# olof3/QuantumOptimalControl.jl

Hardware: AMD Instinct MI355X
Metric: GRAPE gradient evals/sec (dim N, T slices, B seeds) @ 1/2/4/8 GPU (higher is better)
Workload: dtype f64

## Files before the change

quantumoptimalcontrol.jl_amd/csrc/qoc_blkseg.hpp:

```cpp
#pragma once
#include "qoc_blku.hpp"

namespace qoc {

struct BlksegParams {
  double rad[3];
  double mur[3], mui[3];
  double theta_cap;
  int S;
  int L;
  int UPW;
  int RB;
  const double* u;
  double* u_copy;
  double* u_copy2;
  double* J2;
  cx<double>* coef2;
  double* dJdu;
  unsigned long long* terms;
  unsigned int* done;
  double* best;
  long long seed_offset;
  double* best_res;
  double* best_out;
  double2* gseg;
  const int* stale;
  const double2* gtab;
  double pen_mu;
  unsigned int prow[3];
  unsigned int pcol;
  double2* dseg;
};
enum { BLKSEG_FUSED = 0, BLKSEG_FWD = 1, BLKSEG_BWD = 2 };

__host__ __device__ inline size_t blkseg_off_rec(int NB, int nblk) { return (size_t)6 * NB * NB * nblk; }
__host__ __device__ inline size_t blkseg_off_slot(int NB, int nblk, int Nt) { return blkseg_off_rec(NB, nblk) + 4 * (size_t)Nt; }
__host__ __device__ inline size_t blkseg_off_g0(int NB, int nblk, int Nt, int S) {
  return blkseg_off_slot(NB, nblk, Nt) + (size_t)2 * S * NB * NB * nblk;
}
__host__ __device__ inline size_t blkseg_off_xN(int NB, int nblk, int Nt, int S) {
  return blkseg_off_g0(NB, nblk, Nt, S) + (size_t)2 * NB * NB * nblk;
}
__host__ __device__ inline size_t blkseg_off_xt(int N, int m, int NB, int nblk, int Nt, int S) {
  return blkseg_off_xN(NB, nblk, Nt, S) + (size_t)2 * N * m;
}
__host__ __device__ inline size_t blkseg_off_cf(int N, int m, int NB, int nblk, int Nt, int S) {
  return blkseg_off_xt(N, m, NB, nblk, Nt, S) + (size_t)2 * N * m;
}
// ... 17 lines not shown
constexpr size_t BLKSEG_LDS_MAX = (size_t)160 * 1024;
__host__ __device__ inline int blkseg_rb(int upw, int nu) {
  const int r = 64 / (upw * (nu > 0 ? nu : 1));
  return r < 1 ? 1 : r > 4 ? 4 : r;
}

#ifdef QOC_PROBE
static __device__ unsigned long long g_segw[32];
#define SEGW_SET(slot, v)                                                        \
  do {                                                                           \
    if (blockIdx.x == 7 && (threadIdx.x & 63) == 0) g_segw[slot] = (v);          \
  } while (0)
static __device__ int g_seg_noturn, g_seg_turnmode;
#define SEG_TURNS (!g_seg_noturn)
#define SEG_TURNMODE g_seg_turnmode
#else
#define SEG_TURNS true
#define SEG_TURNMODE 1
#define SEGW_SET(slot, v) \
  do {                    \
  } while (0)
#endif


template <int NB, bool AH, bool BH>
__device__ __forceinline__ void seg_mm(const double (&ar)[NB * NB], const double (&ai)[NB * NB], const double (&br)[NB * NB],
                                       const double (&bi)[NB * NB], double (&cr)[NB * NB], double (&ci)[NB * NB]) {
#pragma unroll
  for (int i = 0; i < NB; ++i)
#pragma unroll
    for (int k = 0; k < NB; ++k) {
      double sr = 0.0, si = 0.0;
#pragma unroll
      for (int q = 0; q < NB; ++q) {
        const int ea = AH ? q * NB + i : i * NB + q, eb = BH ? k * NB + q : q * NB + k;
// ... 218 lines not shown
  st = T.s[K];
#pragma unroll
  for (int k = K - 1; k >= 0; --k) {
    ct = fma(ct, t2, T.c[k]);
    st = fma(st, t2, T.s[k]);
  }
  st *= t;
}
template <int K = BLKSEG_KMAX>
__device__ __forceinline__ void sk2_z(const Sk2& g0, const double* rec, double& zr, double& zi) {
  double ct, st;
  sk2_phase<K>(g0.d0, g0.d1, ct, st);
  const double2 ph = *reinterpret_cast<const double2*>(rec);
  zr = ph.x * ct - ph.y * st;
  zi = fma(ph.x, st, ph.y * ct);
}
template <int K = BLKSEG_KMAX, bool EX = false>
__device__ __forceinline__ void sk2_form(const Sk2 (&g)[3], double2 ph, double2 u, Sk2& ah, double (&ur)[4],
                                         double (&ui)[4], double* ex = nullptr) {
  constexpr BlksegTrig T = blkseg_trig();
  ah.d0 = fma(u.y, g[2].d0, fma(u.x, g[1].d0, g[0].d0));
  ah.d1 = fma(u.y, g[2].d1, fma(u.x, g[1].d1, g[0].d1));
  ah.r = fma(u.y, g[2].r, fma(u.x, g[1].r, g[0].r));
  ah.q = fma(u.y, g[2].q, fma(u.x, g[1].q, g[0].q));
  const double a = 0.5 * (ah.d0 - ah.d1);
  const double w = fma(a, a, fma(ah.r, ah.r, ah.q * ah.q));
  double cw = T.c[K], sw = T.s[K], s3 = EX ? T.d[K] : 0.0, ct, st;
#pragma unroll
  for (int k = K - 1; k >= 0; --k) {
    cw = fma(cw, w, T.c[k]);
// ... 262 lines not shown
    Lr[e] = Rr[e] = er * vr - ei * vi;
    Li[e] = Ri[e] = fma(er, vi, ei * vr);
  }
  acc1 = acc2 = 0.0;
  seg_trace<NB>(genf(), Lr, Li, 1.0, m1r, m1i, m2r, m2i, acc1, acc2);
  double f = 1.0;
#pragma unroll 1
  for (int n = 1; n < nex; ++n) {
    seg_rx<NB>(Rr, Ri, xr_, xi_);
    seg_xlr<NB>(Lr, Li, Rr, Ri, xr_, xi_);
    f /= (double)(n + 1);
    seg_trace<NB>(genf(), Lr, Li, f, m1r, m1i, m2r, m2i, acc1, acc2);
  }
}

__device__ __forceinline__ double block_max(double v, double* scratch) {
  for (int off = 32; off > 0; off >>= 1) v = fmax(v, __shfl_xor(v, off));
  const int w = threadIdx.x >> 6, l = threadIdx.x & 63;
  __syncthreads();
  if (l == 0) scratch[w] = v;
  __syncthreads();
  double s = scratch[0];
  const int nw = (blockDim.x + 63) >> 6;
  for (int i = 1; i < nw; ++i) s = fmax(s, scratch[i]);
  __syncthreads();
  return s;
}

__device__ __forceinline__ void wave_lds_sync() {
  __builtin_amdgcn_fence(__ATOMIC_RELEASE, "wavefront");
  __builtin_amdgcn_wave_barrier();
  __builtin_amdgcn_fence(__ATOMIC_ACQUIRE, "wavefront");
}

__device__ __forceinline__ void seg_turn(int grp, int ngrp, int jj) {
  if ((grp + jj) % ngrp == 0) __builtin_amdgcn_s_setprio(1);
  else __builtin_amdgcn_s_setprio(0);
}
template <bool DEFER>
struct SegProg {
  int* prog;
  int partner, other;
  bool on, young;
// ... 57 lines not shown
  }
#pragma unroll
  for (int i = 0; i < NB; ++i)
#pragma unroll
    for (int j = 0; j < NB; ++j) {
      double sr = 0.0, si = 0.0;
#pragma unroll
      for (int q = 0; q < NB; ++q) {
        sr = fma(ur[q * NB + i], tr[q * NB + j], fma(ui[q * NB + i], ti[q * NB + j], sr));
        si = fma(ur[q * NB + i], ti[q * NB + j], fma(-ui[q * NB + i], tr[q * NB + j], si));
      }
      dp[(i * NB + j) * stride] = make_double2(sr, si);
    }
}

template <int NB, int ORD, int WMAX, int MODE = BLKSEG_FUSED, bool PEN = false>
__global__ __launch_bounds__(64 * WMAX) void k_blkseg_eval(const TChainArgs g, const BlkArgs bk, const BlksegParams sp) {
  extern __shared__ __attribute__((aligned(16))) unsigned char smem[];
  if constexpr (MODE == BLKSEG_BWD) {
    if (sp.stale && *sp.stale != 0) return;
  }
  constexpr int E = NB * NB;
  constexpr bool GREG = NB == 2 && WMAX <= 8;
  constexpr bool XA = NB == 2;
  constexpr int NV1 = NB == 2 ? 2 : 1;
  const int N = g.N, m = g.m, nu = g.nu, Nt = g.Nt, nblk = bk.nblk, S = sp.S, L = sp.L;
  const int tid = threadIdx.x, nthr = blockDim.x, w = tid >> 6, l = tid & 63, W = nthr >> 6;
  const int b = blockIdx.x;
  const size_t Nm = (size_t)N * m;
  BK_T(t0);
  double* const lds = reinterpret_cast<double*>(smem);
  double2* const gsh = reinterpret_cast<double2*>(lds);
  double* const rec = lds + blkseg_off_rec(NB, nblk);
  double2* const slot = reinterpret_cast<double2*>(lds + blkseg_off_slot(NB, nblk, Nt));
  double2* const g0s = reinterpret_cast<double2*>(lds + blkseg_off_g0(NB, nblk, Nt, S));
  double* const xN = lds + blkseg_off_xN(NB, nblk, Nt, S);
  double2* const xtl = reinterpret_cast<double2*>(lds + blkseg_off_xt(N, m, NB, nblk, Nt, S));
  cx<double>* const cf = reinterpret_cast<cx<double>*>(lds + blkseg_off_cf(N, m, NB, nblk, Nt, S));
  double* const red = lds + blkseg_off_red(N, m, NB, nblk, Nt, S);
  double* const wred = lds + blkseg_off_wred(N, m, NB, nblk, Nt, S);
  const int RB = sp.RB;
  double* const dJ = lds + blkseg_off_dJ(N, m, NB, nblk, Nt, S, W, RB);
  double2* const d0s = reinterpret_cast<double2*>(lds + blkseg_off_d0(N, m, nu, NB, nblk, Nt, S, W, RB));

  const int uw = l / nblk;
// ... 6 lines not shown
      for (int i = 0; i < NB; ++i) pm |= (int)((sp.prow[i] >> beta) & 1u) << i;
  }
  constexpr int PE = PEN ? NB * NB : 1;
  const int ntab = 3 * E * nblk;
  const double2* const x0g = reinterpret_cast<const double2*>(g.x0) + (g.x0_per_seed ? (size_t)b * Nm : 0);
  const double2* const xtg = reinterpret_cast<const double2*>(g.Xt);
  const double* ub = sp.u + (size_t)b * Nt * nu;
  const bool u16 = nu == 2 && (reinterpret_cast<size_t>(ub) & 15) == 0;
  auto load_u = [&](int k) -> double2 {
    if (u16) return reinterpret_cast<const double2*>(ub)[k];
    return make_double2(nu > 0 ? ub[(size_t)k * nu] : 0.0, nu > 1 ? ub[(size_t)k * nu + 1] : 0.0);
  };
  const bool hasx = MODE != BLKSEG_BWD && (size_t)tid < Nm;
  double2 tab0 = make_double2(0.0, 0.0), x00 = tab0, xt0 = tab0, ua = tab0, ubb = tab0;
  if (tid < ntab) tab0 = sp.gtab[tid];
  if (hasx) {
    x00 = x0g[tid];
    xt0 = xtg[tid];
  }
  if (tid < Nt) ua = load_u(tid);
  if (tid + nthr < Nt) ubb = load_u(tid + nthr);
  int brw[NB];
#pragma unroll
  for (int i = 0; i < NB; ++i) brw[i] = bk.brow[beta * NB + i];
  {
    if (tid < ntab) gsh[tid] = tab0;
    for (int q = tid + nthr; q < ntab; q += nthr) gsh[q] = sp.gtab[q];
    if constexpr (MODE != BLKSEG_BWD) {
      double2* const xN2 = reinterpret_cast<double2*>(xN);
      if (hasx) {
        xN2[tid] = x00;
        xtl[tid] = xt0;
      }
      for (size_t o = (size_t)tid + nthr; o < Nm; o += nthr) {
        xN2[o] = x0g[o];
        xtl[o] = xtg[o];
      }
    }
  }
  double rmax = 0.0;
  const bool cmu = sp.mur[1] == 0.0 && sp.mur[2] == 0.0 && sp.mui[1] == 0.0 && sp.mui[2] == 0.0;
  double2 emu0 = make_double2(1.0, 0.0);
  if (cmu) {
    const double er = exp(sp.mur[0]);
    double sn, cs;
    sincos(sp.mui[0], &sn, &cs);
    emu0 = make_double2(er * cs, er * sn);
  }
  auto slice = [&](int k, double2 uk) {
    const double u1 = uk.x, u2 = uk.y;
    for (int j = 0; j < nu; ++j) {
      const double v = j ? u2 : u1;
      if (sp.u_copy) sp.u_copy[((size_t)b * Nt + k) * nu + j] = v;
      if (sp.u_copy2) sp.u_copy2[((size_t)b * Nt + k) * nu + j] = v;
    }
    rmax = fmax(rmax, fma(fabs(u2), sp.rad[2], fma(fabs(u1), sp.rad[1], sp.rad[0])));
    double2* r = reinterpret_cast<double2*>(rec + 4 * (size_t)k);
    if (cmu) {
      r[0] = emu0;
    } else {
      const double mr = fma(u2, sp.mur[2], fma(u1, sp.mur[1], sp.mur[0]));
      const double mi = fma(u2, sp.mui[2], fma(u1, sp.mui[1], sp.mui[0]));
      const double er = exp(mr);
      double sn, cs;
      sincos(mi, &sn, &cs);
      r[0] = make_double2(er * cs, er * sn);
    }
    r[1] = make_double2(u1, u2);
  };
  if (tid < Nt) slice(tid, ua);
  if (tid + nthr < Nt) slice(tid + nthr, ubb);
  for (int k = tid + 2 * nthr; k < Nt; k += nthr) slice(k, load_u(k));
  rmax = block_max(rmax, red);
  int J = 0;
  double s0 = 1.0;
  while (rmax * s0 > sp.theta_cap && J < 60) {
    s0 *= 0.5;
    ++J;
  }
  int P = 0;
  {
    const double bb = rmax * s0, tol = 1.1102230246251565e-16;
    constexpr BlkuCoef K = blku_coef();
    double term = bb;
#pragma unroll
    for (int q = 0; q < BLKU_TMAX; ++q) {
      if (!(term > tol * fma(-bb, K.inv[q + 2], 1.0))) break;
      P = q + 1;
      term *= bb * K.inv[q + 2];
    }
  }
  P = __builtin_amdgcn_readfirstlane(P);
  J = __builtin_amdgcn_readfirstlane(J);
  int nex = 1;
  if constexpr (ORD == 0) nex = __builtin_amdgcn_readfirstlane(blkseg_exact_terms(rmax));
  if (tid < 8) reinterpret_cast<int*>(red + 24)[tid] = 0;
  if (J) {
    for (int k = tid; k < Nt; k += nthr) {
      rec[4 * (size_t)k + 2] *= s0;
      rec[4 * (size_t)k + 3] *= s0;
    }
  }
  __syncthreads();
  BK_T(t1);
  BK_ADD(0, t1 - t0);

  const int s = w * sp.UPW + uw;
  const bool sact = lact && s < S;
  const int kb = sact ? s * L : 0;
  const int ke = sact ? min(kb + L, Nt) : 0;
  double2 greg[GREG ? 3 : 1][GREG ? E : 1];
  if constexpr (GREG) {
#pragma unroll
    for (int j = 0; j < 3; ++j)
#pragma unroll
      for (int e = 0; e < E; ++e) greg[j][e] = gsh[(beta * 3 + j) * E + e];
  }
  auto gen_at = [&](int bc) {
// ... 24 lines not shown
  double Hr[PE], Hi[PE];
#pragma unroll
  for (int e = 0; e < PE; ++e) Hr[e] = Hi[e] = 0.0;
  const int Lf = Nt - (S - 1) * L;
  const bool fast = NB == 2 && J == 0;
  Sk2 gk[3];
  if constexpr (NB == 2) {
#pragma unroll
    for (int j = 0; j < 3; ++j) {
      double2 e4[4];
#pragma unroll
      for (int e = 0; e < 4; ++e) e4[e] = gsh[(beta * 3 + j) * E + e];
      gk[j] = sk2_of(e4);
    }
  }
  const bool zdl = NB != 2 || (gk[1].d0 == 0.0 && gk[1].d1 == 0.0 && gk[2].d0 == 0.0 && gk[2].d1 == 0.0);
  const bool zd = __syncthreads_and(zdl ? 1 : 0) != 0 && cmu && sp.mur[0] == 0.0;
  const double za0 = NB == 2 ? 0.5 * (gk[0].d0 - gk[0].d1) : 0.0;
  const int ksel = __builtin_amdgcn_readfirstlane(blkseg_series_k(rmax * s0));
  const bool su = fast && zd;
  double pq[4] = {1.0, 0.0, 0.0, 0.0};
  auto lane_z = [&](double& zr, double& zi) {
    zr = 1.0;
    zi = 0.0;
    if constexpr (NB == 2) {
      if (su) {
        if (ksel == 5) sk2_z<5>(gk[0], rec, zr, zi);
        else if (ksel == 7) sk2_z<7>(gk[0], rec, zr, zi);
        else sk2_z<BLKSEG_KMAX>(gk[0], rec, zr, zi);
      }
    }
  };
  const double* const reck = rec + 4 * (size_t)kb;
  auto p1_fast = [&](int jj, auto SEL_, auto K_, auto ZD_) {
    constexpr bool SEL = decltype(SEL_)::value;
    constexpr int KS = decltype(K_)::value;
    constexpr bool ZD = decltype(ZD_)::value;
    if constexpr (NB == 2) {
    if constexpr (ZD) {
      double vv[2][4];
      bool act[2];
#pragma unroll
      for (int v = 0; v < 2; ++v) {
        const int k = kb + jj + v;
// ... 57 lines not shown
      p1_fast(jj, std::true_type(), K_, ZD_);
    }
    if constexpr (NB == 2) {
      if constexpr (decltype(ZD_)::value) sk2_expand(pq, qr, qi);
    }
  };
  auto loop1 = [&](auto K_) {
    if (zd) loop1z(K_, std::true_type());
    else loop1z(K_, std::false_type());
  };
  double Gr[E], Gi[E];
  auto gseg_at = [&](int e) -> double2& { return sp.gseg[(((size_t)b * E + e) * S + s) * nblk + beta]; };
  auto dl_at = [&](int e) -> double2& { return slot[((size_t)s * E + e) * nblk + beta]; };
  auto dseg_at = [&](int e) -> double2& { return sp.dseg[(((size_t)b * E + e) * S + s) * nblk + beta]; };
  if constexpr (MODE == BLKSEG_BWD) {
#pragma unroll
    for (int e = 0; e < E; ++e) {
      const double2 v = sact ? gseg_at(e) : make_double2(0.0, 0.0);
      Gr[e] = v.x;
      Gi[e] = v.y;
    }
    if constexpr (PEN) {
      if (pm)
#pragma unroll
        for (int e = 0; e < E; ++e) dl_at(e) = dseg_at(e);
    }
    if (sp.coef2 && tid < 2 * m) sp.coef2[(size_t)b * 2 * m + tid] = g.coef[(size_t)b * 2 * m + tid];
  } else {
  if (fast) {
    if (ksel == 5) loop1(std::integral_constant<int, 5>());
// ... 53 lines not shown
#pragma unroll
            for (int q = 0; q < NB; ++q) {
              dr[a * NB + q] = fma(xr[a], xr[q], fma(xi[a], xi[q], dr[a * NB + q]));
              di[a * NB + q] = fma(xi[a], xr[q], fma(-xr[a], xi[q], di[a * NB + q]));
            }
        }
#pragma unroll
      for (int e = 0; e < E; ++e) d0s[e * nblk + beta] = make_double2(dr[e], di[e]);
    }
  }

  if (turns || sprog.on) __builtin_amdgcn_s_setprio(0);
  BK_T(t2);
  BK_ADD(1, t2 - t1);
  SEGW_SET(w, t2 - t0);
  auto slot_at = [&](int ss, int e) -> double2& { return slot[((size_t)ss * E + e) * nblk + beta]; };
  const int UPW = sp.UPW, uw0 = lact ? uw : 0;
  if (sact)
#pragma unroll
    for (int e = 0; e < E; ++e) slot_at(s, e) = make_double2(qr[e], qi[e]);
  wave_lds_sync();
  for (int d = 1; d < UPW; d <<= 1) {
    const bool take = sact && uw0 >= d;
    double tr[E], ti[E];
#pragma unroll
    for (int e = 0; e < E; ++e) {
      const double2 v = take ? slot_at(s - d, e) : make_double2(0.0, 0.0);
      tr[e] = v.x;
      ti[e] = v.y;
    }
    wave_lds_sync();
    if (take) {
      double cr[E], ci[E];
      seg_mm<NB, false, false>(qr, qi, tr, ti, cr, ci);
#pragma unroll
      for (int e = 0; e < E; ++e) {
        qr[e] = cr[e];
        qi[e] = ci[e];
        slot_at(s, e) = make_double2(cr[e], ci[e]);
      }
    }
    wave_lds_sync();
  }
  lds_barrier();
  if (sact && w > 0) {
    double er[E], ei[E];
#pragma unroll
    for (int e = 0; e < E; ++e) {
      const double2 v = slot_at(UPW - 1, e);
      er[e] = v.x;
      ei[e] = v.y;
    }
    for (int v = 1; v < w; ++v) {
      double tr[E], ti[E], cr[E], ci[E];
#pragma unroll
      for (int e = 0; e < E; ++e) {
        const double2 x = slot_at(v * UPW + UPW - 1, e);
        tr[e] = x.x;
        ti[e] = x.y;
// ... 8 lines not shown
    double cr[E], ci[E];
    seg_mm<NB, false, false>(qr, qi, er, ei, cr, ci);
#pragma unroll
    for (int e = 0; e < E; ++e) {
      qr[e] = cr[e];
      qi[e] = ci[e];
    }
  }
  if constexpr (PEN) {
    if (pm) {
      double tr[E], ti[E];
      seg_mm<NB, true, false>(qr, qi, Hr, Hi, tr, ti);
      seg_mm<NB, false, false>(tr, ti, qr, qi, Hr, Hi);
    }
  }
  const bool last = sact && s == S - 1;
  if (last) {
    double znr = 1.0, zni = 0.0;
    if (su) {
      double br, bi;
      lane_z(br, bi);
      for (int n = Nt; n > 0; n >>= 1) {
        if (n & 1) {
          const double t = znr * br - zni * bi;
          zni = fma(znr, bi, zni * br);
          znr = t;
        }
        const double t = br * br - bi * bi;
        bi = 2.0 * (br * bi);
        br = t;
      }
    }
    for (int c = 0; c < m; ++c) {
      double xr[NB], xi[NB];
#pragma unroll
      for (int i = 0; i < NB; ++i) {
        const size_t o = 2 * ((size_t)c * N + max(brw[i], 0));
        xr[i] = brw[i] >= 0 ? xN[o] : 0.0;
        xi[i] = brw[i] >= 0 ? xN[o + 1] : 0.0;
      }
#pragma unroll
      for (int i = 0; i < NB; ++i) {
        double yr = 0.0, yi = 0.0;
#pragma unroll
        for (int q = 0; q < NB; ++q) {
          yr = fma(qr[i * NB + q], xr[q], fma(-qi[i * NB + q], xi[q], yr));
          yi = fma(qr[i * NB + q], xi[q], fma(qi[i * NB + q], xr[q], yi));
        }
        if (su) {
          const double t = yr * znr - yi * zni;
          yi = fma(yr, zni, yi * znr);
          yr = t;
        }
        if (brw[i] >= 0) {
          const size_t o = 2 * ((size_t)c * N + brw[i]);
          xN[o] = yr;
          xN[o + 1] = yi;
        }
      }
    }
  }
  __syncthreads();
  if constexpr (PEN) {
    if (pm)
#pragma unroll
      for (int e = 0; e < E; ++e) slot_at(s, e) = make_double2(Hr[e], Hi[e]);
    wave_lds_sync();
    for (int d = 1; d < UPW; d <<= 1) {
      const bool take = pm && uw0 + d < UPW && s + d < S;
      double tr[E], ti[E];
#pragma unroll
      for (int e = 0; e < E; ++e) {
        const double2 v = take ? slot_at(s + d, e) : make_double2(0.0, 0.0);
        tr[e] = v.x;
        ti[e] = v.y;
      }
      wave_lds_sync();
      if (take) {
#pragma unroll
        for (int e = 0; e < E; ++e) {
          Hr[e] += tr[e];
          Hi[e] += ti[e];
          slot_at(s, e) = make_double2(Hr[e], Hi[e]);
        }
      }
      wave_lds_sync();
    }
  }
  chain_costs<double>(N, m, reinterpret_cast<const cx<double>*>(xtl), [&](int q) { return cx<double>{xN[2 * q], xN[2 * q + 1]}; },
                      g.cost_kind, g.n_norm, 0.0, red, red + 16, cf, g.sc);
  __syncthreads();
  if (tid < 2 * m) {
    g.coef[(size_t)b * 2 * m + tid] = cf[tid];
    if (sp.coef2) sp.coef2[(size_t)b * 2 * m + tid] = cf[tid];
  }
  auto later_waves = [&](double (&ar)[E], double (&ai)[E]) {
#pragma unroll
    for (int e = 0; e < E; ++e) ar[e] = ai[e] = 0.0;
    for (int v = w + 1; v < W; ++v)
#pragma unroll
      for (int e = 0; e < E; ++e) {
        const double2 x = slot_at(v * UPW, e);
        ar[e] += x.x;
        ai[e] += x.y;
      }
  };
  if constexpr (PEN) {
    double pj = 0.0;
    if (pm && s == 0) {
      double ar[E], ai[E];
      later_waves(ar, ai);
#pragma unroll
      for (int a = 0; a < NB; ++a)
#pragma unroll
        for (int q = 0; q < NB; ++q) {
          const double2 d0 = d0s[(a * NB + q) * nblk + beta], h = slot_at(0, q * NB + a);
          const double mr = h.x + ar[q * NB + a] + (a == q && ((pm >> a) & 1) ? 1.0 : 0.0);
          const double mi = h.y + ai[q * NB + a];
          pj = fma(d0.x, mr, fma(-d0.y, mi, pj));
        }
    }
    if (w == 0) {
      if (l < nblk) wred[l] = pj;
      wave_lds_sync();
    }
  }
  if (tid == 0) {
    double Jv = red[16];
    if constexpr (PEN) {
      double ps = 0.0;
      for (int q = 0; q < nblk; ++q) ps += wred[q];
      Jv = fma(sp.pen_mu, ps, Jv);
    }
    __hip_atomic_store(reinterpret_cast<unsigned long long*>(g.J + b),
                       (unsigned long long)__double_as_longlong(Jv), __ATOMIC_RELAXED, __HIP_MEMORY_SCOPE_AGENT);
    if (sp.J2) sp.J2[b] = Jv;
  }
#if defined(__HIP_DEVICE_COMPILE__) && !defined(__gfx950__)
#error "k_blkseg_eval's best-(J, seed) hand-off is written for gfx950"
#endif
  const bool early = W <= 4;
  auto publish = [&]() {
    if (w != 0 || !sp.done) return;
    unsigned int prev = 0;
    if (l == 0) {
      asm volatile("s_waitcnt vmcnt(0)" ::: "memory");
      prev = __hip_atomic_fetch_add(sp.done, 1u, __ATOMIC_RELAXED, __HIP_MEMORY_SCOPE_AGENT);
    }
    prev = __shfl(prev, 0);
    if (prev == gridDim.x - 1) {
      __builtin_amdgcn_fence(__ATOMIC_ACQUIRE, "agent");
      asm volatile("s_waitcnt vmcnt(0)" ::: "memory");
// ... 19 lines not shown
        const double bs = bi >= 0 ? (double)(bi + sp.seed_offset) : -1.0;
        sp.best[0] = bv;
        sp.best[1] = bs;
        if (sp.best_res) {
          sp.best_res[0] = bv;
          sp.best_res[1] = bs;
        }
        if (sp.best_out) {
          sp.best_out[0] = bv;
          sp.best_out[1] = bs;
        }
        *sp.done = 0;
      }
    }
  };
  if (early) publish();
  if (last) {
    const cx<double>* Xt = reinterpret_cast<const cx<double>*>(xtl);
    double gr[E], gi[E];
#pragma unroll
    for (int e = 0; e < E; ++e) gr[e] = gi[e] = 0.0;
    for (int c = 0; c < m; ++c) {
      double2 xv[NB], lv[NB];
#pragma unroll
      for (int i = 0; i < NB; ++i) {
        const int r = brw[i];
        const size_t o = (size_t)c * N + max(r, 0);
        const cx<double> f = lam_coef(cf, g.sc, m, max(r, 0), c), t = Xt[o];
        xv[i] = r >= 0 ? make_double2(xN[2 * o], xN[2 * o + 1]) : make_double2(0.0, 0.0);
        lv[i] = r >= 0 ? make_double2(f.r * t.r - f.i * t.i, f.r * t.i + f.i * t.r) : make_double2(0.0, 0.0);
      }
      blku_kacc<NB>(gr, gi, xv, lv);
    }
    double tr[E], ti[E], cr[E], ci[E];
    seg_mm<NB, true, false>(qr, qi, gr, gi, tr, ti);
    seg_mm<NB, false, false>(tr, ti, qr, qi, cr, ci);
#pragma unroll
    for (int e = 0; e < E; ++e) g0s[e * nblk + beta] = make_double2(cr[e], ci[e]);
  }
  if constexpr (PEN) {
    if (pm) {
      later_waves(Hr, Hi);
      if (uw0 + 1 < UPW && s + 1 < S)
#pragma unroll
        for (int e = 0; e < E; ++e) {
          const double2 x = slot_at(s + 1, e);
          Hr[e] += x.x;
          Hi[e] += x.y;
        }
    }
  }
  __syncthreads();
  {
    double hr[E], hi[E], tr[E], ti[E];
#pragma unroll
    for (int e = 0; e < E; ++e) {
      const double2 v = g0s[e * nblk + beta];
      hr[e] = v.x;
      hi[e] = v.y;
    }
    if constexpr (PEN) {
      if (pm) {
        double dr[E], di[E];
#pragma unroll
        for (int e = 0; e < E; ++e) {
          const double2 v = d0s[e * nblk + beta];
          dr[e] = v.x;
// ... 23 lines not shown
#pragma unroll
            for (int q = 0; q < NB; ++q) {
              sr = fma(dr[i * NB + q], Hr[q * NB + j], fma(-di[i * NB + q], Hi[q * NB + j], sr));
              si = fma(dr[i * NB + q], Hi[q * NB + j], fma(di[i * NB + q], Hr[q * NB + j], si));
            }
            hr[i * NB + j] = fma(f, sr, hr[i * NB + j]);
            hi[i * NB + j] = fma(f, si, hi[i * NB + j]);
          }
        __builtin_amdgcn_sched_barrier(0);
      }
    }
    seg_mm<NB, false, false>(qr, qi, hr, hi, tr, ti);
    seg_mm<NB, false, true>(tr, ti, qr, qi, Gr, Gi);
  }

  if (!early) publish();
  BK_T(t2e);
  BK_ADD(2, t2e - t2);
  if constexpr (MODE == BLKSEG_FWD) {
    if (sact)
#pragma unroll
      for (int e = 0; e < E; ++e) gseg_at(e) = make_double2(Gr[e], Gi[e]);
    if (sp.terms && tid == 0) atomicAdd(sp.terms + b % TERM_SLOTS, (unsigned long long)Nt * ((unsigned long long)P << J));
    return;
  }
  }
  BK_T(t3);
  const double mu1r = sp.mur[1], mu1i = sp.mui[1], mu2r = sp.mur[2], mu2i = sp.mui[2];
  const double pen2 = PEN ? 2.0 * sp.pen_mu : 0.0;
  auto pen_step = [&](const double (&ur)[E], const double (&ui)[E]) {
    seg_pen_step<NB>(pm, pen2, slot + (size_t)opaque(s) * E * nblk + beta, nblk, ur, ui, Gr, Gi);
  };
  double zr, zi;
  lane_z(zr, zi);
  if (su) {
#pragma unroll
    for (int e = 0; e < E; ++e) {
      const double t = fma(zr, Gr[e], zi * Gi[e]);
      Gi[e] = fma(zr, Gi[e], -zi * Gr[e]);
      Gr[e] = t;
    }
  }
  const double pen2r = pen2 * zr, pen2i = -pen2 * zi;
  auto pen_step_v = [&](const double (&ur)[E], const double (&ui)[E]) {
    seg_pen_step<NB, true>(pm, pen2r, slot + (size_t)opaque(s) * E * nblk + beta, nblk, ur, ui, Gr, Gi, pen2i);
  };
  double* const wr = wred + 128 * RB * w;
  const int nrl = sp.UPW * max(nu, 1);
  const int rq = l / nrl, rrem = l - rq * nrl, ro = rrem / max(nu, 1), rj = rrem - ro * max(nu, 1);
// ... 159 lines not shown
        const double2* const gp = slot + (size_t)opaque(sact ? s : 0) * E * nblk + beta;
#pragma unroll
        for (int e = 0; e < E; ++e) {
          const double2 v = gp[e * nblk];
          Gr[e] = v.x;
          Gi[e] = v.y;
        }
      }
      reduce(jj, act ? acc1 : 0.0, act ? acc2 : 0.0);
    }
  }
  if (turns || sprog.on) __builtin_amdgcn_s_setprio(0);
  BK_T(t4);
  BK_ADD(3, t4 - t3);
  SEGW_SET(16 + w, t4 - t0);
  __syncthreads();
  double* const og = sp.dJdu + (size_t)b * Nt * nu;
  for (int i = tid; i < Nt * nu; i += nthr) og[i] = dJ[i];
  if (MODE == BLKSEG_FUSED && sp.terms && tid == 0)
    atomicAdd(sp.terms + b % TERM_SLOTS, (unsigned long long)Nt * ((unsigned long long)P << J));
  BK_T(t5);
  BK_ADD(4, t5 - t4);
  BK_ADD(5, t5 - t0);
}

}
```

quantumoptimalcontrol.jl_amd/csrc/qoc_chain.hpp:

```cpp
#pragma once
#include "qoc_common.hpp"
#include "qoc_expm.hpp"

namespace qoc {

constexpr int CHAIN_THREADS = 256;

struct ChainShape {
  int S, JT, CB;
};
__host__ __device__ inline int chain_groups(int N, int S) {
  const int G = (N + 64 / S - 1) / (64 / S);
  return G == 1 ? 4 : G == 2 ? 2 : 1;
}
__host__ __device__ inline ChainShape chain_shape(int N, int m, bool fp64) {
  const int S = N <= 16 ? 4 : N <= 32 ? 8 : 4;
  const int cpw = (m + chain_groups(N, S) - 1) / chain_groups(N, S);
  const int cb = cpw >= 4 ? 4 : 1;
  if (N <= 32) return {S, 4, cb};
  const int J = (N + 3) / 4;
  return {4, J <= 10 ? 10 : J <= 12 ? 12 : (fp64 ? 0 : 16), m >= 2 ? 2 : 1};
}
template <typename T>
constexpr int chain_max_n() {
// ... 163 lines not shown
          coef[sc.zmap[c]] = v;
        } else {
          coef[c] = v;
          coef[m + c] = v;
        }
      }
    }
  } else {
    if (tid == 0) {
      *Jout = psum;
      for (int c = 0; c < 2 * m; ++c) coef[c] = cx<double>{0, 0};
    }
  }
}

template <typename T>
__global__ void k_terminal_cost(int N, int m, int Nt, const cx<T>* __restrict__ X, const cx<T>* __restrict__ Xt,
                                int cost_kind, double n_norm, int accumulate, double* __restrict__ J,
                                cx<double>* __restrict__ coef, Sectors sc) {
  __shared__ double red[8];
  const int b = blockIdx.x;
  const size_t Nm = (size_t)N * m;
  const cx<T>* xN = X + ((size_t)b * (Nt + 1) + Nt) * Nm;
  const double psum = accumulate ? J[b] : 0.0;
  __syncthreads();
  chain_costs<T>(N, m, Xt, [&](int o) { return xN[o]; }, cost_kind, n_norm, psum, red, J + b,
                 coef + (size_t)b * 2 * m, sc);
}

template <typename T>
// ... 434 lines not shown
```

quantumoptimalcontrol.jl_amd/csrc/qoc_internal.hpp:

```cpp
#pragma once
#include <hip/hip_runtime.h>

#include <algorithm>
#include <cmath>
#include <cstdarg>
#include <cstdio>
#include <cstdlib>
#include <cstring>
#include <initializer_list>
#include <string>
#include <type_traits>
#include <vector>

#include "../../include/qoc.h"
#include "qoc_chain.hpp"
#include "qoc_comm.hpp"
#include "qoc_tchain.hpp"

namespace qoc {
struct BlkArgs;
}
using namespace qoc;

struct BlksegShape {
// ... 308 lines not shown
int blkp_forward(qoc_ctx* c);
bool blkp_backward_ok(const qoc_ctx* c, int order);
int blkp_backward(qoc_ctx* c, int order, double* d_dJdu, const int* stale);

int blku_forward(qoc_ctx* c);
int blku_backward(qoc_ctx* c, int order, double* d_dJdu);
int blku_eval_concurrent(qoc_ctx* c, int order, double* d_dJdu);
int blku_states(qoc_ctx* c);
int blku_costates(qoc_ctx* c);

bool blkseg_ok(const qoc_ctx* c, int order);
int blkseg_eval(qoc_ctx* c, int order, const double* d_u, double* d_J, double* d_dJdu);
bool blkseg_split_ok(const qoc_ctx* c);
int blkseg_forward(qoc_ctx* c, const double* d_u, double* d_J);
int blkseg_backward(qoc_ctx* c, int order, double* d_dJdu, const int* stale);

}
```

quantumoptimalcontrol.jl_amd/csrc/qoc_run_blk.hip:

```cpp
#include <numeric>

#include "qoc_blk_host.hpp"

namespace qoc_host {

int blk_detect(qoc_ctx* c) {
  c->blk_nb = 0;
  c->nblk = 0;
  c->blk_jr = 0;
  c->blk_real = false;
  c->nwb = 0;
  c->h_brow.clear();
  c->seg_pen_valid = false;
  if (env_is("QOC_BLOCKS", "0")) return QOC_OK;
  const bool valu = env_is("QOC_BLOCKS", "valu");
  const bool real_req = env_is("QOC_BLOCKS", "real");
  const int N = c->N;
  const size_t NN = (size_t)N * N;
  std::vector<int> par(N);
  std::iota(par.begin(), par.end(), 0);
  auto find = [&](int x) {
    while (par[x] != x) x = par[x] = par[par[x]];
    return x;
  };
// ... 71 lines not shown
    if (*p) {
      HIPCHK(c, hipFree(*p));
      *p = nullptr;
    }
  c->dev_bytes -= c->blk_dev_bytes;
  c->blk_dev_bytes = 0;
  HIPCHK(c, hipMalloc((void**)&c->d_brow, brow.size() * sizeof(int)));
  HIPCHK(c, hipMemcpy(c->d_brow, brow.data(), brow.size() * sizeof(int), hipMemcpyHostToDevice));
  c->blk_dev_bytes += brow.size() * sizeof(int);
  if (c->d_gtab) {
    HIPCHK(c, hipFree(c->d_gtab));
    c->d_gtab = nullptr;
  }
  if (NB <= 3) {
    const int E = NB * NB;
    std::vector<double> tab((size_t)nblk * 3 * E * 2, 0.0);
    for (int b = 0; b < nblk; ++b)
      for (int j = 0; j <= c->nu && j < 3; ++j)
        for (int e = 0; e < E; ++e) {
          const int ri = brow[(size_t)b * NB + e / NB], rk = brow[(size_t)b * NB + e % NB];
          if (ri < 0 || rk < 0) continue;
          const double* v = c->h_gen.data() + 2 * (j * NN + ri + (size_t)N * rk);
          double* t = tab.data() + 2 * (((size_t)b * 3 + j) * E + e);
          t[0] = ri == rk ? v[0] - c->tprm.mur[j] : v[0];
          t[1] = ri == rk ? v[1] - c->tprm.mui[j] : v[1];
        }
    HIPCHK(c, hipMalloc((void**)&c->d_gtab, tab.size() * sizeof(double)));
    HIPCHK(c, hipMemcpy(c->d_gtab, tab.data(), tab.size() * sizeof(double), hipMemcpyHostToDevice));
    c->blk_dev_bytes += tab.size() * sizeof(double);
  }
  if (jr || real) {
    HIPCHK(c, hipMalloc((void**)&c->d_wrow, wrow.size() * sizeof(int)));
    HIPCHK(c, hipMemcpy(c->d_wrow, wrow.data(), wrow.size() * sizeof(int), hipMemcpyHostToDevice));
    c->blk_dev_bytes += wrow.size() * sizeof(int);
  }
  c->dev_bytes += c->blk_dev_bytes;
  c->blk_nb = NB;
  c->nblk = nblk;
  c->blk_jr = jr;
  c->blk_real = real;
  c->nwb = (int)(wrow.size() / 16);
  return QOC_OK;
}

bool blk_active(const qoc_ctx* c) {
  if (c->blk_nb <= 0 || c->prec != QOC_FP64 || c->chain_mode != 1 || c->prop_method != QOC_PROP_EXPM || c->big ||
      c->packed || c->nu > 2)
    return false;
  if (c->blk_real) return c->nwb * ((c->m + 3) / 4) <= 8;
  if (c->blk_jr) return c->nwb * ((c->m + 1) / 2) <= 8 && (c->blk_nb < 16 || tchain_mf(c));
  return c->nblk * c->m <= BLK_MAXT && c->nblk <= 256;
}
bool blk_rot(const qoc_ctx* c) { return c->blk_jr > 0 || c->blk_real; }

bool blku_on(const qoc_ctx* c) {
  if (!blk_active(c) || c->blk_jr != 1 || c->blk_nb > BLK_NBMAX || c->nu < 1 || c->nu > 2 || c->nblk > 32 ||
      c->nblk * c->m * (c->blk_nb == 2 ? 2 : 4) > 64 * (c->blk_nb == 4 ? 2 : 4))
// ... 240 lines not shown
```

quantumoptimalcontrol.jl_amd/csrc/qoc_run_blkseg.hip:

```cpp
#include <cstring>

#include "qoc_blk_host.hpp"
#include "qoc_blkseg.hpp"
#include "qoc_internal.hpp"

namespace qoc_host {

static bool blkseg_pen(const qoc_ctx* c) {
  if (c->mu == 0.0) return false;
  if (!c->seg_pen_valid) {
    c->seg_prow[0] = c->seg_prow[1] = c->seg_prow[2] = 0;
    c->seg_pcol = 0;
    const int NB = c->blk_nb;
    if (NB >= 2 && NB <= 3 && c->nblk <= 32 && (int)c->h_brow.size() == c->nblk * NB)
      for (int r : c->h_pen_rows)
        for (int q = 0; q < c->nblk * NB; ++q)
          if (c->h_brow[q] == r) c->seg_prow[q % NB] |= 1u << (q / NB);
    for (int col : c->h_pen_cols)
      if (col >= 0 && col < 32) c->seg_pcol |= 1u << col;
    c->seg_pen_valid = true;
  }
  return (c->seg_prow[0] | c->seg_prow[1] | c->seg_prow[2]) != 0 && c->seg_pcol != 0;
}

// ... 33 lines not shown
  if (c->mu != 0.0 && (env_is("QOC_BLKSEG_PEN", "0") || c->m > 32)) return false;
  return blkseg_shape(c).lds <= BLKSEG_LDS_MAX;
}

template <typename F>
static hipError_t blkseg_dispatch(int NB, int order, F&& f) {
  if (order == QOC_DUKDP_EXACT) {
    const std::integral_constant<int, 0> ex;
    if (NB == 2) return f(std::integral_constant<int, 2>(), ex);
    return f(std::integral_constant<int, 3>(), ex);
  }
  return blk_order_dispatch(order, [&](auto ORD_) {
    if (NB == 2) return f(std::integral_constant<int, 2>(), ORD_);
    return f(std::integral_constant<int, 3>(), ORD_);
  });
}

static int ensure_lazy_bufs(qoc_ctx* c) {
  const size_t nu_t = (size_t)c->B * c->nu * c->Nt, ncf = (size_t)c->B * 2 * c->m_user;
  if (!c->d_u_lam) {
    HIPCHK(c, hipMalloc((void**)&c->d_u_lam, nu_t * sizeof(double)));
    HIPCHK(c, hipMalloc((void**)&c->d_coef_lam, ncf * sizeof(cx<double>)));
    c->dev_bytes += nu_t * sizeof(double) + ncf * sizeof(cx<double>);
  }
  return QOC_OK;
}

static int blkseg_params(qoc_ctx* c, const BlksegShape& s, BlksegParams& sp) {
  sp = BlksegParams{};
  for (int j = 0; j < 3; ++j) {
// ... 172 lines not shown
```

Baseline: 4.791 million.

## Precompute per-block phase constants and shrink block-wide barriers in blkseg eval

```diff
diff --git a/quantumoptimalcontrol.jl_amd/csrc/qoc_blkseg.hpp b/quantumoptimalcontrol.jl_amd/csrc/qoc_blkseg.hpp
--- a/quantumoptimalcontrol.jl_amd/csrc/qoc_blkseg.hpp
+++ b/quantumoptimalcontrol.jl_amd/csrc/qoc_blkseg.hpp
@@ -32,6 +32,8 @@
   double2* dseg;
 };
 enum { BLKSEG_FUSED = 0, BLKSEG_FWD = 1, BLKSEG_BWD = 2 };
+__host__ __device__ inline size_t blkseg_nconst(int NB, int nblk) { return NB == 2 ? 2 + (size_t)6 * nblk : 0; }
+__host__ __device__ constexpr int blkseg_kclass(int ksel) { return ksel == 5 ? 0 : ksel == 7 ? 1 : 2; }
 
 __host__ __device__ inline size_t blkseg_off_rec(int NB, int nblk) { return (size_t)6 * NB * NB * nblk; }
 __host__ __device__ inline size_t blkseg_off_slot(int NB, int nblk, int Nt) { return blkseg_off_rec(NB, nblk) + 4 * (size_t)Nt; }
@@ -79,11 +81,40 @@
 static __device__ int g_seg_noturn, g_seg_turnmode;
 #define SEG_TURNS (!g_seg_noturn)
 #define SEG_TURNMODE g_seg_turnmode
+static __device__ unsigned long long g_bks[32];
+#define BKS_NOW(var)                                                             \
+  do {                                                                           \
+    __builtin_amdgcn_sched_barrier(0);                                           \
+    asm volatile("s_memtime %0\n\ts_waitcnt lgkmcnt(0)" : "=s"(var)::"memory"); \
+    __builtin_amdgcn_sched_barrier(0);                                           \
+  } while (0)
+#define BKS_INIT unsigned long long bks_prev_ = 0
+#define BKS_MARK BKS_NOW(bks_prev_)
+#define BKS(slot)                                                                                        \
+  do {                                                                                                   \
+    unsigned long long bks_n_;                                                                           \
+    BKS_NOW(bks_n_);                                                                                     \
+    if (blockIdx.x == 7 && (threadIdx.x & 63) == 0) atomicAdd(&g_bks[slot], bks_n_ - bks_prev_);         \
+    bks_prev_ = bks_n_;                                                                                  \
+  } while (0)
+#define BKS_VMWAIT asm volatile("s_waitcnt vmcnt(0)" ::: "memory")
 #else
 #define SEG_TURNS true
 #define SEG_TURNMODE 1
 #define SEGW_SET(slot, v) \
   do {                    \
+  } while (0)
+#define BKS_INIT \
+  do {           \
+  } while (0)
+#define BKS_MARK \
+  do {           \
+  } while (0)
+#define BKS(slot) \
+  do {            \
+  } while (0)
+#define BKS_VMWAIT \
+  do {             \
   } while (0)
 #endif
 
@@ -332,6 +363,20 @@
   const double2 ph = *reinterpret_cast<const double2*>(rec);
   zr = ph.x * ct - ph.y * st;
   zi = fma(ph.x, st, ph.y * ct);
+}
+__device__ __forceinline__ void sk2_zpow(double br, double bi, int n, double& znr, double& zni) {
+  znr = 1.0;
+  zni = 0.0;
+  for (; n > 0; n >>= 1) {
+    if (n & 1) {
+      const double t = znr * br - zni * bi;
+      zni = fma(znr, bi, zni * br);
+      znr = t;
+    }
+    const double t = br * br - bi * bi;
+    bi = 2.0 * (br * bi);
+    br = t;
+  }
 }
 template <int K = BLKSEG_KMAX, bool EX = false>
 __device__ __forceinline__ void sk2_form(const Sk2 (&g)[3], double2 ph, double2 u, Sk2& ah, double (&ur)[4],
@@ -624,19 +669,6 @@
   }
 }
 
-__device__ __forceinline__ double block_max(double v, double* scratch) {
-  for (int off = 32; off > 0; off >>= 1) v = fmax(v, __shfl_xor(v, off));
-  const int w = threadIdx.x >> 6, l = threadIdx.x & 63;
-  __syncthreads();
-  if (l == 0) scratch[w] = v;
-  __syncthreads();
-  double s = scratch[0];
-  const int nw = (blockDim.x + 63) >> 6;
-  for (int i = 1; i < nw; ++i) s = fmax(s, scratch[i]);
-  __syncthreads();
-  return s;
-}
-
 __device__ __forceinline__ void wave_lds_sync() {
   __builtin_amdgcn_fence(__ATOMIC_RELEASE, "wavefront");
   __builtin_amdgcn_wave_barrier();
@@ -724,6 +756,45 @@
     }
 }
 
+__global__ __launch_bounds__(64) void k_blkseg_consts(double2* gtab, int nblk, int Nt, double mur0, double mui0,
+                                                       int cmu) {
+  const int beta = threadIdx.x, bb = beta < nblk ? beta : 0;
+  double2* const ct = gtab + (size_t)12 * nblk;
+  double2 emu0 = make_double2(1.0, 0.0);
+  if (cmu) {
+    const double er = exp(mur0);
+    double sn, cs;
+    sincos(mui0, &sn, &cs);
+    emu0 = make_double2(er * cs, er * sn);
+  }
+  Sk2 gk[3];
+#pragma unroll
+  for (int j = 0; j < 3; ++j) {
+    double2 e4[4];
+#pragma unroll
+    for (int e = 0; e < 4; ++e) e4[e] = gtab[(bb * 3 + j) * 4 + e];
+    gk[j] = sk2_of(e4);
+  }
+  const bool zdl = gk[1].d0 == 0.0 && gk[1].d1 == 0.0 && gk[2].d0 == 0.0 && gk[2].d1 == 0.0;
+  const bool zd = __all(zdl ? 1 : 0) && cmu && mur0 == 0.0;
+  if (beta == 0) {
+    ct[0] = emu0;
+    ct[1] = make_double2(zd ? 1.0 : 0.0, 0.0);
+  }
+  if (beta >= nblk) return;
+  auto put = [&](auto K_) {
+    constexpr int K = decltype(K_)::value;
+    double zr, zi, znr, zni;
+    sk2_z<K>(gk[0], reinterpret_cast<const double*>(&emu0), zr, zi);
+    sk2_zpow(zr, zi, Nt, znr, zni);
+    ct[2 + 2 * (3 * beta + blkseg_kclass(K))] = make_double2(zr, zi);
+    ct[3 + 2 * (3 * beta + blkseg_kclass(K))] = make_double2(znr, zni);
+  };
+  put(std::integral_constant<int, 5>());
+  put(std::integral_constant<int, 7>());
+  put(std::integral_constant<int, BLKSEG_KMAX>());
+}
+
 template <int NB, int ORD, int WMAX, int MODE = BLKSEG_FUSED, bool PEN = false>
 __global__ __launch_bounds__(64 * WMAX) void k_blkseg_eval(const TChainArgs g, const BlkArgs bk, const BlksegParams sp) {
   extern __shared__ __attribute__((aligned(16))) unsigned char smem[];
@@ -739,6 +810,8 @@
   const int b = blockIdx.x;
   const size_t Nm = (size_t)N * m;
   BK_T(t0);
+  BKS_INIT;
+  BKS_MARK;
   double* const lds = reinterpret_cast<double*>(smem);
   double2* const gsh = reinterpret_cast<double2*>(lds);
   double* const rec = lds + blkseg_off_rec(NB, nblk);
@@ -775,6 +848,12 @@
   const bool hasx = MODE != BLKSEG_BWD && (size_t)tid < Nm;
   double2 tab0 = make_double2(0.0, 0.0), x00 = tab0, xt0 = tab0, ua = tab0, ubb = tab0;
   if (tid < ntab) tab0 = sp.gtab[tid];
+  const double2* const ctab = sp.gtab + ntab;
+  double2 cemu = make_double2(1.0, 0.0), czd = make_double2(0.0, 0.0);
+  if constexpr (NB == 2) {
+    cemu = ctab[0];
+    czd = ctab[1];
+  }
   if (hasx) {
     x00 = x0g[tid];
     xt0 = xtg[tid];
@@ -784,6 +863,8 @@
   int brw[NB];
 #pragma unroll
   for (int i = 0; i < NB; ++i) brw[i] = bk.brow[beta * NB + i];
+  BKS_VMWAIT;
+  BKS(0);
   {
     if (tid < ntab) gsh[tid] = tab0;
     for (int q = tid + nthr; q < ntab; q += nthr) gsh[q] = sp.gtab[q];
@@ -802,7 +883,9 @@
   double rmax = 0.0;
   const bool cmu = sp.mur[1] == 0.0 && sp.mur[2] == 0.0 && sp.mui[1] == 0.0 && sp.mui[2] == 0.0;
   double2 emu0 = make_double2(1.0, 0.0);
-  if (cmu) {
+  if constexpr (NB == 2) {
+    if (cmu) emu0 = cemu;
+  } else if (cmu) {
     const double er = exp(sp.mur[0]);
     double sn, cs;
     sincos(sp.mui[0], &sn, &cs);
@@ -832,7 +915,13 @@
   if (tid < Nt) slice(tid, ua);
   if (tid + nthr < Nt) slice(tid + nthr, ubb);
   for (int k = tid + 2 * nthr; k < Nt; k += nthr) slice(k, load_u(k));
-  rmax = block_max(rmax, red);
+  BKS(1);
+  for (int off = 32; off > 0; off >>= 1) rmax = fmax(rmax, __shfl_xor(rmax, off));
+  if (l == 0) red[w] = rmax;
+  lds_barrier();
+  rmax = red[0];
+  for (int i = 1; i < W; ++i) rmax = fmax(rmax, red[i]);
+  BKS(2);
   int J = 0;
   double s0 = 1.0;
   while (rmax * s0 > sp.theta_cap && J < 60) {
@@ -862,7 +951,8 @@
       rec[4 * (size_t)k + 3] *= s0;
     }
   }
-  __syncthreads();
+  lds_barrier();
+  BKS(3);
   BK_T(t1);
   BK_ADD(0, t1 - t0);
 
@@ -917,20 +1007,19 @@
       gk[j] = sk2_of(e4);
     }
   }
-  const bool zdl = NB != 2 || (gk[1].d0 == 0.0 && gk[1].d1 == 0.0 && gk[2].d0 == 0.0 && gk[2].d1 == 0.0);
-  const bool zd = __syncthreads_and(zdl ? 1 : 0) != 0 && cmu && sp.mur[0] == 0.0;
+  const bool zd = NB == 2 ? __builtin_amdgcn_readfirstlane(czd.x != 0.0 ? 1 : 0) != 0 : cmu && sp.mur[0] == 0.0;
   const double za0 = NB == 2 ? 0.5 * (gk[0].d0 - gk[0].d1) : 0.0;
   const int ksel = __builtin_amdgcn_readfirstlane(blkseg_series_k(rmax * s0));
+  BKS(4);
   const bool su = fast && zd;
   double pq[4] = {1.0, 0.0, 0.0, 0.0};
-  auto lane_z = [&](double& zr, double& zi) {
-    zr = 1.0;
-    zi = 0.0;
+  double2 zt = make_double2(1.0, 0.0), znt = zt;
+  auto load_z = [&]() {
     if constexpr (NB == 2) {
       if (su) {
-        if (ksel == 5) sk2_z<5>(gk[0], rec, zr, zi);
-        else if (ksel == 7) sk2_z<7>(gk[0], rec, zr, zi);
-        else sk2_z<BLKSEG_KMAX>(gk[0], rec, zr, zi);
+        const double2* const zp = ctab + 2 + 2 * (3 * beta + blkseg_kclass(ksel));
+        zt = zp[0];
+        znt = zp[1];
       }
     }
   };
@@ -1018,6 +1107,7 @@
   auto dl_at = [&](int e) -> double2& { return slot[((size_t)s * E + e) * nblk + beta]; };
   auto dseg_at = [&](int e) -> double2& { return sp.dseg[(((size_t)b * E + e) * S + s) * nblk + beta]; };
   if constexpr (MODE == BLKSEG_BWD) {
+    load_z();
 #pragma unroll
     for (int e = 0; e < E; ++e) {
       const double2 v = sact ? gseg_at(e) : make_double2(0.0, 0.0);
@@ -1101,6 +1191,8 @@
   BK_T(t2);
   BK_ADD(1, t2 - t1);
   SEGW_SET(w, t2 - t0);
+  BKS_MARK;
+  load_z();
   auto slot_at = [&](int ss, int e) -> double2& { return slot[((size_t)ss * E + e) * nblk + beta]; };
   const int UPW = sp.UPW, uw0 = lact ? uw : 0;
   if (sact)
@@ -1129,7 +1221,9 @@
     }
     wave_lds_sync();
   }
+  BKS(5);
   lds_barrier();
+  BKS(6);
   if (sact && w > 0) {
     double er[E], ei[E];
 #pragma unroll
@@ -1168,23 +1262,11 @@
       seg_mm<NB, false, false>(tr, ti, qr, qi, Hr, Hi);
     }
   }
+  BKS(7);
   const bool last = sact && s == S - 1;
-  if (last) {
-    double znr = 1.0, zni = 0.0;
-    if (su) {
-      double br, bi;
-      lane_z(br, bi);
-      for (int n = Nt; n > 0; n >>= 1) {
-        if (n & 1) {
-          const double t = znr * br - zni * bi;
-          zni = fma(znr, bi, zni * br);
-          znr = t;
-        }
-        const double t = br * br - bi * bi;
-        bi = 2.0 * (br * bi);
-        br = t;
-      }
-    }
+  auto xn_step = [&]() {
+    if (!last) return;
+    const double znr = znt.x, zni = znt.y;
     for (int c = 0; c < m; ++c) {
       double xr[NB], xi[NB];
 #pragma unroll
@@ -1213,9 +1295,9 @@
         }
       }
     }
-  }
-  __syncthreads();
-  if constexpr (PEN) {
+  };
+  auto pen_suffix = [&]() {
+    if constexpr (PEN) {
     if (pm)
 #pragma unroll
       for (int e = 0; e < E; ++e) slot_at(s, e) = make_double2(Hr[e], Hi[e]);
@@ -1240,14 +1322,14 @@
       }
       wave_lds_sync();
     }
-  }
-  chain_costs<double>(N, m, reinterpret_cast<const cx<double>*>(xtl), [&](int q) { return cx<double>{xN[2 * q], xN[2 * q + 1]}; },
-                      g.cost_kind, g.n_norm, 0.0, red, red + 16, cf, g.sc);
-  __syncthreads();
-  if (tid < 2 * m) {
-    g.coef[(size_t)b * 2 * m + tid] = cf[tid];
-    if (sp.coef2) sp.coef2[(size_t)b * 2 * m + tid] = cf[tid];
-  }
+    }
+  };
+  auto coef_out = [&](int t, int nt) {
+    for (int q = t; q < 2 * m; q += nt) {
+      g.coef[(size_t)b * 2 * m + q] = cf[q];
+      if (sp.coef2) sp.coef2[(size_t)b * 2 * m + q] = cf[q];
+    }
+  };
   auto later_waves = [&](double (&ar)[E], double (&ai)[E]) {
 #pragma unroll
     for (int e = 0; e < E; ++e) ar[e] = ai[e] = 0.0;
@@ -1259,7 +1341,8 @@
         ai[e] += x.y;
       }
   };
-  if constexpr (PEN) {
+  auto pen_share = [&]() {
+    if constexpr (PEN) {
     double pj = 0.0;
     if (pm && s == 0) {
       double ar[E], ai[E];
@@ -1278,8 +1361,10 @@
       if (l < nblk) wred[l] = pj;
       wave_lds_sync();
     }
-  }
-  if (tid == 0) {
+    }
+  };
+  auto j_store = [&](bool mine) {
+    if (!mine) return;
     double Jv = red[16];
     if constexpr (PEN) {
       double ps = 0.0;
@@ -1289,7 +1374,7 @@
     __hip_atomic_store(reinterpret_cast<unsigned long long*>(g.J + b),
                        (unsigned long long)__double_as_longlong(Jv), __ATOMIC_RELAXED, __HIP_MEMORY_SCOPE_AGENT);
     if (sp.J2) sp.J2[b] = Jv;
-  }
+  };
 #if defined(__HIP_DEVICE_COMPILE__) && !defined(__gfx950__)
 #error "k_blkseg_eval's best-(J, seed) hand-off is written for gfx950"
 #endif
@@ -1339,8 +1424,8 @@
       }
     }
   };
-  if (early) publish();
-  if (last) {
+  auto gn_step = [&]() {
+    if (!last) return;
     const cx<double>* Xt = reinterpret_cast<const cx<double>*>(xtl);
     double gr[E], gi[E];
 #pragma unroll
@@ -1362,6 +1447,51 @@
     seg_mm<NB, false, false>(tr, ti, qr, qi, cr, ci);
 #pragma unroll
     for (int e = 0; e < E; ++e) g0s[e * nblk + beta] = make_double2(cr[e], ci[e]);
+  };
+  const int wl = (S - 1) / UPW;
+  const auto xn_at = [&](int q) { return cx<double>{xN[2 * q], xN[2 * q + 1]}; };
+  if (!early) {
+    if constexpr (PEN) {
+      lds_barrier();
+      BKS(9);
+      pen_suffix();
+    }
+    if (__builtin_amdgcn_readfirstlane(w) == wl) {
+      xn_step();
+      BKS(8);
+      wave_lds_sync();
+      chain_costs_wave<double>(N, m, reinterpret_cast<const cx<double>*>(xtl), xn_at, g.cost_kind, g.n_norm, 0.0, nthr,
+                               red + 16, cf, g.sc);
+      wave_lds_sync();
+      BKS(10);
+      coef_out(l, 64);
+      BKS(11);
+      if constexpr (!PEN) j_store(l == 0);
+      gn_step();
+      if constexpr (!PEN) asm volatile("s_waitcnt vmcnt(0)" ::: "memory");
+    }
+    if constexpr (PEN) {
+      lds_barrier();
+      pen_share();
+    }
+  } else {
+    xn_step();
+    BKS(8);
+    __syncthreads();
+    BKS(9);
+    pen_suffix();
+    chain_costs<double>(N, m, reinterpret_cast<const cx<double>*>(xtl), xn_at, g.cost_kind, g.n_norm, 0.0, red, red + 16,
+                        cf, g.sc);
+    BKS(10);
+    __syncthreads();
+    coef_out(tid, nthr);
+    BKS(11);
+    pen_share();
+    if (early) {
+      j_store(tid == 0);
+      publish();
+    }
+    gn_step();
   }
   if constexpr (PEN) {
     if (pm) {
@@ -1375,7 +1505,10 @@
         }
     }
   }
-  __syncthreads();
+  BKS(12);
+  lds_barrier();
+  BKS(13);
+  if (PEN && !early) j_store(tid == 0);
   {
     double hr[E], hi[E], tr[E], ti[E];
 #pragma unroll
@@ -1429,7 +1562,9 @@
     seg_mm<NB, false, true>(tr, ti, qr, qi, Gr, Gi);
   }
 
+  BKS(14);
   if (!early) publish();
+  BKS(15);
   BK_T(t2e);
   BK_ADD(2, t2e - t2);
   if constexpr (MODE == BLKSEG_FWD) {
@@ -1446,8 +1581,7 @@
   auto pen_step = [&](const double (&ur)[E], const double (&ui)[E]) {
     seg_pen_step<NB>(pm, pen2, slot + (size_t)opaque(s) * E * nblk + beta, nblk, ur, ui, Gr, Gi);
   };
-  double zr, zi;
-  lane_z(zr, zi);
+  const double zr = zt.x, zi = zt.y;
   if (su) {
 #pragma unroll
     for (int e = 0; e < E; ++e) {
@@ -1637,11 +1771,28 @@
   BK_T(t4);
   BK_ADD(3, t4 - t3);
   SEGW_SET(16 + w, t4 - t0);
-  __syncthreads();
-  double* const og = sp.dJdu + (size_t)b * Nt * nu;
-  for (int i = tid; i < Nt * nu; i += nthr) og[i] = dJ[i];
+  BKS_MARK;
+  BKS(16);
+  if constexpr (NB != 2) {
+    __syncthreads();
+    double* const og = sp.dJdu + (size_t)b * Nt * nu;
+    for (int i = tid; i < Nt * nu; i += nthr) og[i] = dJ[i];
+  } else {
+    const int k0 = min(w * sp.UPW * L, Nt), k1 = min(k0 + sp.UPW * L, Nt);
+    const int i0 = k0 * nu, n = (k1 - k0) * nu;
+    double* const og = sp.dJdu + (size_t)b * Nt * nu + i0;
+    const double* const src = dJ + i0;
+    if (((src - lds) & 1) == 0 && (reinterpret_cast<size_t>(og) & 15) == 0) {
+      for (int i = 2 * l; i + 1 < n; i += 128)
+        *reinterpret_cast<double2*>(og + i) = *reinterpret_cast<const double2*>(src + i);
+      if ((n & 1) && l == 0) og[n - 1] = src[n - 1];
+    } else {
+      for (int i = l; i < n; i += 64) og[i] = src[i];
+    }
+  }
   if (MODE == BLKSEG_FUSED && sp.terms && tid == 0)
     atomicAdd(sp.terms + b % TERM_SLOTS, (unsigned long long)Nt * ((unsigned long long)P << J));
+  BKS(17);
   BK_T(t5);
   BK_ADD(4, t5 - t4);
   BK_ADD(5, t5 - t0);
diff --git a/quantumoptimalcontrol.jl_amd/csrc/qoc_chain.hpp b/quantumoptimalcontrol.jl_amd/csrc/qoc_chain.hpp
--- a/quantumoptimalcontrol.jl_amd/csrc/qoc_chain.hpp
+++ b/quantumoptimalcontrol.jl_amd/csrc/qoc_chain.hpp
@@ -201,6 +201,102 @@
   }
 }
 
+template <typename T, typename XN>
+__device__ __forceinline__ void chain_costs_wave(int N, int m, const cx<T>* __restrict__ Xt, XN&& xN, int cost_kind,
+                                                 double n_norm, double psum, int nthr, double* Jout,
+                                                 cx<double>* __restrict__ coef, const Sectors& sc = Sectors()) {
+  const int l = threadIdx.x & 63, nw = (nthr + 63) >> 6, Nm = N * m;
+  auto sums = [&](int n, auto&& f, double& sr, double& si) {
+    sr = 0.0;
+    si = 0.0;
+    for (int p0 = 0; p0 < nw; p0 += 4) {
+      double a[4], c[4];
+#pragma unroll
+      for (int q = 0; q < 4; ++q) a[q] = c[q] = 0;
+      if (64 * p0 < n) {
+#pragma unroll
+        for (int q = 0; q < 4; ++q) {
+          const int o = 64 * (p0 + q) + l;
+          if (p0 + q < nw && o < n) f(o, a[q], c[q]);
+        }
+#pragma unroll
+        for (int off = 32; off > 0; off >>= 1) {
+          double ta[4], tc[4];
+#pragma unroll
+          for (int q = 0; q < 4; ++q) {
+            ta[q] = __shfl_xor(a[q], off);
+            tc[q] = __shfl_xor(c[q], off);
+          }
+#pragma unroll
+          for (int q = 0; q < 4; ++q) {
+            a[q] += ta[q];
+            c[q] += tc[q];
+          }
+        }
+      }
+#pragma unroll
+      for (int q = 0; q < 4; ++q)
+        if (p0 + q < nw) {
+          sr += a[q];
+          si += c[q];
+        }
+    }
+  };
+  if (cost_kind == COST_TRACE) {
+    double orr, oii;
+    sums(Nm, [&](int o, double& a, double& c) {
+      const cx<T> t = Xt[o], v = xN(o);
+      a += (double)t.r * v.r + (double)t.i * v.i;
+      c += (double)t.r * v.i - (double)t.i * v.r;
+    }, orr, oii);
+    if (l == 0) {
+      const double n2 = n_norm * n_norm;
+      *Jout = 1.0 - fma(orr, orr, oii * oii) / n2 + psum;
+      for (int c = 0; c < 2 * m; ++c) coef[c] = cx<double>{-2.0 * orr / n2, -2.0 * oii / n2};
+    }
+  } else if (cost_kind == COST_ZCAL) {
+    cx<double> mm[4];
+    for (int c = 0; c < 4; ++c) {
+      const int s = sc.rsec ? sc.zmap[c] / m : -1, col = sc.rsec ? sc.zmap[c] % m : c;
+      sums(N, [&](int i, double& a, double& d) {
+        if (s >= 0 && sc.rsec[i] != s) return;
+        const cx<T> t = Xt[i + N * col], v = xN(i + N * col);
+        a += (double)t.r * v.r + (double)t.i * v.i;
+        d += (double)t.r * v.i - (double)t.i * v.r;
+      }, mm[c].r, mm[c].i);
+    }
+    if (l == 0) {
+      double F, th;
+      optimal_calibration(mm, 1e-9, &F, &th);
+      *Jout = 1.0 - F * F / 16.0 + psum;
+      const cx<double> e = {cos(th), sin(th)}, em = {cos(th), -sin(th)};
+      const cx<double> v1 = {mm[0].r + e.r * mm[1].r - e.i * mm[1].i, mm[0].i + e.r * mm[1].i + e.i * mm[1].r};
+      const cx<double> v2 = {mm[2].r + e.r * mm[3].r - e.i * mm[3].i, mm[2].i + e.r * mm[3].i + e.i * mm[3].r};
+      const double a1 = sqrt(v1.r * v1.r + v1.i * v1.i), a2 = sqrt(v2.r * v2.r + v2.i * v2.i);
+      const cx<double> g[4] = {{v1.r / a1, v1.i / a1},
+                               {(v1.r * em.r - v1.i * em.i) / a1, (v1.r * em.i + v1.i * em.r) / a1},
+                               {v2.r / a2, v2.i / a2},
+                               {(v2.r * em.r - v2.i * em.i) / a2, (v2.r * em.i + v2.i * em.r) / a2}};
+      const double sc2 = -2.0 * F / 16.0;
+      for (int c = 0; c < 2 * m; ++c) coef[c] = cx<double>{0, 0};
+      for (int c = 0; c < 4; ++c) {
+        const cx<double> v = {sc2 * g[c].r, sc2 * g[c].i};
+        if (sc.rsec) {
+          coef[sc.zmap[c]] = v;
+        } else {
+          coef[c] = v;
+          coef[m + c] = v;
+        }
+      }
+    }
+  } else {
+    if (l == 0) {
+      *Jout = psum;
+      for (int c = 0; c < 2 * m; ++c) coef[c] = cx<double>{0, 0};
+    }
+  }
+}
+
 template <typename T>
 __global__ void k_terminal_cost(int N, int m, int Nt, const cx<T>* __restrict__ X, const cx<T>* __restrict__ Xt,
                                 int cost_kind, double n_norm, int accumulate, double* __restrict__ J,
diff --git a/quantumoptimalcontrol.jl_amd/csrc/qoc_internal.hpp b/quantumoptimalcontrol.jl_amd/csrc/qoc_internal.hpp
--- a/quantumoptimalcontrol.jl_amd/csrc/qoc_internal.hpp
+++ b/quantumoptimalcontrol.jl_amd/csrc/qoc_internal.hpp
@@ -346,5 +346,7 @@
 bool blkseg_split_ok(const qoc_ctx* c);
 int blkseg_forward(qoc_ctx* c, const double* d_u, double* d_J);
 int blkseg_backward(qoc_ctx* c, int order, double* d_dJdu, const int* stale);
-
-}
+size_t blkseg_table_consts(int nb, int nblk);
+int blkseg_fill_consts(qoc_ctx* c);
+
+}
diff --git a/quantumoptimalcontrol.jl_amd/csrc/qoc_run_blk.hip b/quantumoptimalcontrol.jl_amd/csrc/qoc_run_blk.hip
--- a/quantumoptimalcontrol.jl_amd/csrc/qoc_run_blk.hip
+++ b/quantumoptimalcontrol.jl_amd/csrc/qoc_run_blk.hip
@@ -109,7 +109,7 @@
   }
   if (NB <= 3) {
     const int E = NB * NB;
-    std::vector<double> tab((size_t)nblk * 3 * E * 2, 0.0);
+    std::vector<double> tab(((size_t)nblk * 3 * E + blkseg_table_consts(NB, nblk)) * 2, 0.0);
     for (int b = 0; b < nblk; ++b)
       for (int j = 0; j <= c->nu && j < 3; ++j)
         for (int e = 0; e < E; ++e) {
@@ -135,7 +135,7 @@
   c->blk_jr = jr;
   c->blk_real = real;
   c->nwb = (int)(wrow.size() / 16);
-  return QOC_OK;
+  return blkseg_fill_consts(c);
 }
 
 bool blk_active(const qoc_ctx* c) {
diff --git a/quantumoptimalcontrol.jl_amd/csrc/qoc_run_blkseg.hip b/quantumoptimalcontrol.jl_amd/csrc/qoc_run_blkseg.hip
--- a/quantumoptimalcontrol.jl_amd/csrc/qoc_run_blkseg.hip
+++ b/quantumoptimalcontrol.jl_amd/csrc/qoc_run_blkseg.hip
@@ -71,6 +71,21 @@
     if (NB == 2) return f(std::integral_constant<int, 2>(), ORD_);
     return f(std::integral_constant<int, 3>(), ORD_);
   });
+}
+
+size_t blkseg_table_consts(int nb, int nblk) { return nblk <= 32 ? blkseg_nconst(nb, nblk) : 0; }
+
+int blkseg_fill_consts(qoc_ctx* c) {
+  if (!c->d_gtab || blkseg_table_consts(c->blk_nb, c->nblk) == 0) return QOC_OK;
+  double mur[3], mui[3];
+  for (int j = 0; j < 3; ++j) {
+    mur[j] = j <= c->nu ? c->tprm.mur[j] : 0.0;
+    mui[j] = j <= c->nu ? c->tprm.mui[j] : 0.0;
+  }
+  const int cmu = mur[1] == 0.0 && mur[2] == 0.0 && mui[1] == 0.0 && mui[2] == 0.0;
+  hipLaunchKernelGGL(k_blkseg_consts, dim3(1), dim3(64), 0, c->stream, c->d_gtab, c->nblk, c->Nt, mur[0], mui[0], cmu);
+  HIPCHK(c, hipGetLastError());
+  return QOC_OK;
 }
 
 static int ensure_lazy_bufs(qoc_ctx* c) {
```

Result: no change. 4.766 million (-0.5%).
